# Jackxiini/Tensorflow-distributed-learning

Measured on AMD Instinct MI355X. Metric: images/sec (whole node) MNIST CNN global_batch=64*N, higher is better.
Workload: dtype fp32; 1 GPU; global_batch=64, parallelism=dp1, engine=fused, communicator=local, variant=reference, process_model=single, communicator_impl=LocalCommunicator, ipc_mode=dmabuf, allreduce=local, steps_per_execution=25, graph_captured=True, input_prefetch_executions=1, allreduce_in_graph=False, replicas_identical=True

## Files before the change

### csrc/kernels/mnist_cnn.hip

```cpp
#include <type_traits>

#include "common.h"
#include "mnist_cnn.h"
#include "optim.h"
#include "xgmi_device.h"

namespace tdl {

struct HeadWeights {
  float wa[10], wb[10], b4[10], b3a, b3b;
};

__device__ __forceinline__ HeadWeights load_head_weights(const MnistArgs& a, int l) {
  HeadWeights hw;
  const float* w4 = a.W + a.ow4;
#pragma unroll
  for (int c = 0; c < 10; ++c) {
    hw.wa[c] = w4[l * 10 + c];
    hw.wb[c] = w4[(l + 64) * 10 + c];
    hw.b4[c] = a.W[a.ob4 + c];
  }
  hw.b3a = a.W[a.ob3 + l];
  hw.b3b = a.W[a.ob3 + l + 64];
  return hw;
// ... 493 lines not shown
#pragma unroll
  for (int j = 0; j < 10; ++j) dw[j] = 0.f;
  const int d = 7 - wave;
  const int pix0 = half ? kDgSplit : 0, pix1 = half ? 169 : kDgSplit;
  if (d < (pix1 - pix0 + 15) / 16) {
    const int P = pix0 + d * 16 + i;
    const bool valid = P < pix1;
    const int Pc = valid ? P : pix0;
    const int ih = Pc / 13, iw = Pc - ih * 13;
    const float* wb = Wd + (g * 16 + i) * 4;
    const int c = 16 * h + i;
    unsigned q1v[4];
#pragma unroll
    for (int r = 0; r < 4; ++r) {
      const int Pr = min(pix0 + d * 16 + 4 * g + r, pix1 - 1);
      q1v[r] = a.A1[((size_t)bi * 169 + Pr) * 32 + c];
    }
    const int ih_lo = (pix0 + d * 16) / 13, ih_hi = min(pix0 + d * 16 + 15, pix1 - 1) / 13;
    const int kh_lo = max(0, ih_lo - 9), kh_hi = min(2, ih_hi);
    f4 acc0 = zero4(), acc1 = zero4();
    for (int kh = kh_lo; kh <= kh_hi; ++kh) {
#pragma unroll
      for (int kw = 0; kw < 3; ++kw) {
        const int tap = kh * 3 + kw;
        const float* ap = dCs + ((ih - kh + 2) * kDcDim + (iw - kw + 2)) * kDcStride + 4 * g;
#pragma unroll
        for (int c0 = 0; c0 < 64; c0 += 16) {
          const f4 av = ld4(ap + c0);
          const f4 bv = ld4(wb + (tap * 16 + c0 / 4) * 64);
          acc0 = mfma16x16x4(av.x, bv.x, acc0);
          acc1 = mfma16x16x4(av.y, bv.y, acc1);
          acc0 = mfma16x16x4(av.z, bv.z, acc0);
          acc1 = mfma16x16x4(av.w, bv.w, acc1);
        }
      }
    }
    const f4 acc = acc0 + acc1;
    stamp(a.stamps, 6);
#pragma unroll
    for (int r = 0; r < 4; ++r) {
      const int Pr = pix0 + d * 16 + 4 * g + r;
      if (Pr < pix1) {
        const float v = P1s[Pr * kP1StrideB + c] > 0.f ? acc[r] : 0.f;
        const unsigned q1 = q1v[r];
        const int ph = Pr / 13, pw = Pr - ph * 13;
        const float* img = Xs + (2 * ph + (q1 >> 1)) * 28 + 2 * pw + (q1 & 1);
#pragma unroll
        for (int kh = 0; kh < 3; ++kh)
#pragma unroll
          for (int kw = 0; kw < 3; ++kw) dw[kh * 3 + kw] = fmaf(img[kh * 28 + kw], v, dw[kh * 3 + kw]);
        dw[9] += v;
      }
    }
  }
#pragma unroll
  for (int j = 0; j < 10; ++j) dw[j] = sum_lane_groups(dw[j]);
  if (g == 0) {
#pragma unroll
    for (int j = 0; j < 10; ++j) red[(wave * 10 + j) * 16 + i] = dw[j];
  }
  stamp(a.stamps, 4);
  __syncthreads();
  stamp(a.stamps, 5);
  if (tid < 160) {
    const int j = tid >> 4, ii = tid & 15;
    float s = 0.f;
#pragma unroll
    for (int w = 2; w < 8; ++w) s += red[(w * 10 + j) * 16 + ii];
    a.part1[((size_t)bi * 2 + half) * kMnistPart1Cols + j * 32 + 16 * h + ii] = s;
  }
}

constexpr int kLdsFwd = 784 + 320 + 169 * kP1Stride + 72 * 16 * 4 + 400 + 169 * 32 / 4 + 400 / 4 + 16 * 128 + 4 + 128 +
                        288 * 16 +
                        kHeadW;
constexpr int kDcF = 15, kDcFStride = 20;
constexpr int kLdsFwdFused = kLdsFwd + kDcF * kDcF * kDcFStride;
constexpr int kP1Live = 12;
constexpr int kConv1Tiles = kP1Live * kP1Live / 4;
__constant__ int kFusedWgradTiles[8][2] = {{0, 2}, {3, 2}, {7, 3}, {12, 3}, {2, 1}, {5, 2}, {10, 2}, {15, 3}};

__device__ __forceinline__ void bwd_stamp(unsigned long long* buf, int k) {
  if (buf != nullptr && (threadIdx.x & 63) == 0)
    buf[(size_t)gridDim.x * 72 + (blockIdx.x * 8 + (threadIdx.x >> 6)) * 4 + k] = __builtin_amdgcn_s_memrealtime();
}

__device__ __forceinline__ void dgrad_mfma_stamp(unsigned long long* buf) {
#ifdef TDL_DIAG_DGRAD_STAMP
  if (buf != nullptr && (threadIdx.x & 63) == 0)
    buf[(size_t)gridDim.x * 104 + kFxBlocks * 16 + blockIdx.x * 8 + (threadIdx.x >> 6)] = __builtin_amdgcn_s_memrealtime();
#endif
}

constexpr int kWgS = 3;
struct FusedBwdPre {
  int wga[3], wgb;
  float wav[kWgS][3];
  int dga[3], xo[3][4];
  float p1v[3][4];
};

__device__ __forceinline__ int wg_wrap_a(int g) { return g >= 2 ? 3 * kP1Stride : 0; }

__device__ __forceinline__ void fused_bwd_pre(FusedBwdPre& pre, const float* P1s, const uint8_t* a1s) {
  const int wave = __builtin_amdgcn_readfirstlane(threadIdx.x >> 6), lane = threadIdx.x & 63;
  const int i = lane & 15, g = lane >> 4;
  const int t0 = kFusedWgradTiles[wave][0];
#pragma unroll
  for (int u = 0; u < 3; ++u) {
    const int k = min(t0 + u, 17) * 16 + i;
    const int tap = k >> 5, ci = k & 31;
    const int kh = tap / 3, kw = tap - kh * 3;
    pre.wga[u] = (kh * 13 + kw + g) * kP1Stride + ci;
  }
  pre.wgb = (2 * kDcF + 2 + g) * kDcFStride + i;
#pragma unroll
  for (int j = 0; j < kWgS; ++j) {
    const int q = (4 * j) / 10, r = (4 * j) % 10;
#pragma unroll
    for (int u = 0; u < 3; ++u) pre.wav[j][u] = P1s[pre.wga[u] + (q * 13 + r) * kP1Stride + (r == 8 ? wg_wrap_a(g) : 0)];
  }
  const int nt = wave >> 2, wt = wave & 3, ci = 16 * nt + i;
#pragma unroll
  for (int u = 0; u < 3; ++u) {
    const int t = wt + 4 * u;
    const int Pc = min(t * 16 + i, 168);
    const int ih = Pc / 13, iw = Pc - ih * 13;
    pre.dga[u] = ((ih + 2) * kDcF + iw + 2) * kDcFStride + 4 * g;
#pragma unroll
    for (int r = 0; r < 4; ++r) {
      const int Pr = min(t * 16 + 4 * g + r, 168);
      pre.p1v[u][r] = P1s[Pr * kP1Stride + ci];
      const int q1 = a1s[Pr * 32 + ci];
      const int ph = Pr / 13, pw = Pr - ph * 13;
      pre.xo[u][r] = (2 * ph + (q1 >> 1)) * 28 + 2 * pw + (q1 & 1);
    }
  }
}

template <int N>
__device__ __forceinline__ void fused_wgrad_tiles(const MnistArgs& a, int bi, int cq, int t0, const float* P1s,
                                                  const float* dCs, const FusedBwdPre& pre) {
  const int lane = threadIdx.x & 63, i = lane & 15, g = lane >> 4;
  const float* pa0[N];
#pragma unroll
  for (int u = 0; u < N; ++u) pa0[u] = P1s + pre.wga[u];
  const int wrapA = wg_wrap_a(g), wrapB = g >= 2 ? 5 * kDcFStride : 0;
  const float* pb0 = dCs + pre.wgb;
  f4 acc[N];
#pragma unroll
  for (int u = 0; u < N; ++u) acc[u] = zero4();
  constexpr int kS = kWgS, kBlocks = (25 + kS - 1) / kS;
  float bv[2][kS], av[2][kS][N];
  auto load = [&](int buf, int blk) {
#pragma unroll
    for (int j = 0; j < kS; ++j) {
      const int st = blk * kS + j;
      if (st >= 25) break;
      const int q = (4 * st) / 10, r = (4 * st) % 10;
      const bool strad = r == 8;
      bv[buf][j] = pb0[(q * kDcF + r) * kDcFStride + (strad ? wrapB : 0)];
#pragma unroll
      for (int u = 0; u < N; ++u)
        av[buf][j][u] = blk == 0 ? pre.wav[j][u] : pa0[u][(q * 13 + r) * kP1Stride + (strad ? wrapA : 0)];
    }
  };
  load(0, 0);
#pragma unroll
  for (int blk = 0; blk < kBlocks; ++blk) {
    if (blk + 1 < kBlocks) load((blk + 1) & 1, blk + 1);
    __builtin_amdgcn_sched_barrier(0);
#pragma unroll
    for (int j = 0; j < kS; ++j) {
      if (blk * kS + j >= 25) break;
#pragma unroll
      for (int u = 0; u < N; ++u) acc[u] = mfma16x16x4(av[blk & 1][j][u], bv[blk & 1][j], acc[u]);
    }
    __builtin_amdgcn_sched_barrier(0);
  }
  const auto rs = buf_rsrc(a.part2 + (size_t)bi * kP2QuadFloats, kP2QuadFloats * 4);
#pragma unroll
  for (int u = 0; u < N; ++u) st4_sc1(rs, ((((t0 + u) * 4 + g) * 64 + 16 * cq + i) * 4) * 4, acc[u]);
}

__device__ __forceinline__ void lds_dgrad_w2(const float* w2d, f4 (&bwd)[9]) {
  const int wave = __builtin_amdgcn_readfirstlane(threadIdx.x >> 6), lane = threadIdx.x & 63;
  const int i = lane & 15, g = lane >> 4, nt = wave >> 2;
#pragma unroll
  for (int tap = 0; tap < 9; ++tap) bwd[tap] = ld4(w2d + (tap * 32 + 16 * nt + i) * 16 + 4 * g);
}

constexpr int dg_kh_lo(int t) { return (16 * t) / 13 > 9 ? (16 * t) / 13 - 9 : 0; }
constexpr int dg_kh_hi(int t) { return (16 * t + 15) / 13 < 2 ? (16 * t + 15) / 13 : 2; }
constexpr int dg_taps(int t) { return 3 * (dg_kh_hi(t) - dg_kh_lo(t) + 1); }
static_assert(dg_taps(2) == 9 && dg_taps(3) == 9 && dg_taps(6) == 9 && dg_taps(7) == 9, "tile class 2");
static_assert(dg_taps(0) == 6 && dg_taps(4) == 9 && dg_taps(8) == 9 && dg_taps(1) == 9 && dg_taps(5) == 9 &&
              dg_taps(9) == 3, "tile classes 0 and 1");

#define TDL_SGB(mask, n) __builtin_amdgcn_sched_group_barrier(mask, n, 0)

template <int WTC>
__device__ __forceinline__ void fused_dgrad(const FusedBwdPre& pre, const float* dCs, const float* xs,
                                            const f4 (&bwd)[9], float (&dw)[10], unsigned long long* stamps) {
  constexpr int kT = WTC < 2 ? 3 : 2;
  auto lda = [&](int u, int tap) {
    const int kh = tap / 3, kw = tap - kh * 3;
    return ld4(dCs + pre.dga[u] - (kh * kDcF + kw) * kDcFStride);
  };
  auto ldx = [&](int u, int k, int r) { return xs[pre.xo[u][r] + (k / 3) * 28 + k % 3]; };
  f4 acc0 = zero4(), acc1 = zero4(), pacc0 = zero4(), pacc1 = zero4();
  float v[4] = {0.f, 0.f, 0.f, 0.f};
  f4 av[2];
  float ev[2][12];
  float el[9][4];
  av[0] = lda(0, 3 * dg_kh_lo(WTC));
  auto tile = [&](auto uc, auto sc) {
    constexpr int u = decltype(uc)::value, t = WTC + 4 * u, up = u > 0 ? u - 1 : 0;
    constexpr int s0 = decltype(sc)::value;
    constexpr int tap0 = 3 * dg_kh_lo(t), nA = dg_taps(t);
    constexpr int cps = u > 0 ? 9 / nA : 0;
    constexpr int lps = u + 1 == kT ? 9 / nA : 0;
    static_assert((u == 0 || cps * nA == 9) && (u + 1 < kT || lps * nA == 9), "epilogue split over the taps");
    acc0 = zero4();
    acc1 = zero4();
#pragma unroll
    for (int j = 0; j < nA; ++j) {
      const int p = (s0 + j) & 1;
      if (j + 1 < nA) {
        av[p ^ 1] = lda(u, tap0 + j + 1);
#pragma unroll
        for (int e = 0; e < 4 * cps; ++e) ev[p ^ 1][e] = ldx(up, (j + 1) * cps + (e >> 2), e & 3);
      } else if constexpr (u + 1 < kT) {
        constexpr int ncps = 9 / dg_taps(t + 4);
        av[p ^ 1] = lda(u + 1, 3 * dg_kh_lo(t + 4));
#pragma unroll
        for (int e = 0; e < 4 * ncps; ++e) ev[p ^ 1][e] = ldx(u, e >> 2, e & 3);
      }
#pragma unroll
      for (int e = 0; e < 4 * lps; ++e) el[j * lps + (e >> 2)][e & 3] = ldx(u, j * lps + (e >> 2), e & 3);
      __builtin_amdgcn_sched_barrier(0);
      const f4 x = av[p], bv = bwd[tap0 + j];
      auto fmas = [&](int first, int n) {
#pragma unroll
        for (int e = first; e < first + n; ++e) {
          const int k = j * cps + (e >> 2);
          dw[k] = fmaf(ev[p][e], v[e & 3], dw[k]);
        }
      };
      if (u > 0 && j == 0) {
        acc0 = mfma16x16x4(x.x, bv.x, acc0);
        acc1 = mfma16x16x4(x.y, bv.y, acc1);
        const f4 ac = pacc0 + pacc1;
#pragma unroll
        for (int r = 0; r < 4; ++r) {
          v[r] = pre.p1v[up][r] > 0.f ? ac[r] : 0.f;
          dw[9] += v[r];
        }
        acc0 = mfma16x16x4(x.z, bv.z, acc0);
        fmas(0, 2 * cps);
        acc1 = mfma16x16x4(x.w, bv.w, acc1);
        fmas(2 * cps, 2 * cps);
        TDL_SGB(0x8, 2);
        TDL_SGB(0x2, 16);
        TDL_SGB(0x8, 1);
        TDL_SGB(0x2, 2 * cps);
        TDL_SGB(0x8, 1);
        TDL_SGB(0x2, 2 * cps);
      } else {
        acc0 = mfma16x16x4(x.x, bv.x, acc0);
        fmas(0, cps);
        acc1 = mfma16x16x4(x.y, bv.y, acc1);
        fmas(cps, cps);
        acc0 = mfma16x16x4(x.z, bv.z, acc0);
        fmas(2 * cps, cps);
        acc1 = mfma16x16x4(x.w, bv.w, acc1);
        fmas(3 * cps, cps);
        if constexpr (cps > 0) {
#pragma unroll
          for (int m = 0; m < 4; ++m) {
            TDL_SGB(0x8, 1);
            TDL_SGB(0x2, cps);
          }
        }
      }
      __builtin_amdgcn_sched_barrier(0);
    }
    pacc0 = acc0;
    pacc1 = acc1;
  };
  constexpr int n0 = dg_taps(WTC), n1 = dg_taps(WTC + 4);
  tile(std::integral_constant<int, 0>{}, std::integral_constant<int, 0>{});
  tile(std::integral_constant<int, 1>{}, std::integral_constant<int, n0>{});
  if constexpr (kT == 3) tile(std::integral_constant<int, 2>{}, std::integral_constant<int, n0 + n1>{});
  dgrad_mfma_stamp(stamps);
  const f4 ac = pacc0 + pacc1;
#pragma unroll
  for (int r = 0; r < 4; ++r) {
    const float vl = pre.p1v[kT - 1][r] > 0.f ? ac[r] : 0.f;
#pragma unroll
    for (int k = 0; k < 9; ++k) dw[k] = fmaf(el[k][r], vl, dw[k]);
    dw[9] += vl;
  }
}
#undef TDL_SGB

__device__ __forceinline__ void fused_conv_bwd(const MnistArgs& a, int bi, int cq, const float* dp2s,
                                               const uint8_t* a2s, const float* P1s, const uint8_t* a1s,
                                               const float* xs, float* dCs, float* red, const f4 (&bwd)[9],
                                               FusedBwdPre& pre) {
  const int tid = threadIdx.x, wave = __builtin_amdgcn_readfirstlane(tid >> 6), lane = tid & 63;
  const int i = lane & 15, g = lane >> 4;
  bwd_stamp(a.stamps, 0);
  if (wave == 0) fused_bwd_pre(pre, P1s, a1s);

  auto wgrad = [&]() {
    const int t0 = kFusedWgradTiles[wave][0], ntiles = kFusedWgradTiles[wave][1];
    if (ntiles == 2) fused_wgrad_tiles<2>(a, bi, cq, t0, P1s, dCs, pre);
    else if (ntiles == 3) fused_wgrad_tiles<3>(a, bi, cq, t0, P1s, dCs, pre);
    else fused_wgrad_tiles<1>(a, bi, cq, t0, P1s, dCs, pre);
  };
  const bool swap = (a.variant & kMnistVariantStagger) && wave >= 4;
  if (!swap) wgrad();
  bwd_stamp(a.stamps, 1);

  float dw[10];
#pragma unroll
  for (int j = 0; j < 10; ++j) dw[j] = 0.f;
  const int wt = wave & 3;
  if (wt == 0) fused_dgrad<0>(pre, dCs, xs, bwd, dw, a.stamps);
  else if (wt == 1) fused_dgrad<1>(pre, dCs, xs, bwd, dw, a.stamps);
  else fused_dgrad<2>(pre, dCs, xs, bwd, dw, a.stamps);
  if (swap) wgrad();
  bwd_stamp(a.stamps, 2);
#pragma unroll
  for (int j = 0; j < 10; ++j) dw[j] = sum_lane_groups(dw[j]);
  if (g == 0) {
#pragma unroll
    for (int j = 0; j < 10; ++j) red[(wave * 10 + j) * 16 + i] = dw[j];
  }
  lds_barrier();
  bwd_stamp(a.stamps, 3);
  if (tid < kMnistPart1Cols) {
    const int j = tid >> 5, c = tid & 31, nt = c >> 4, ii = c & 15;
    float sum = 0.f;
#pragma unroll
    for (int w = 0; w < 4; ++w) sum += red[((4 * nt + w) * 10 + j) * 16 + ii];
    a.part1[((size_t)bi * 4 + cq) * kMnistPart1Cols + tid] = sum;
  }
}

__device__ __forceinline__ void store_saved_fwd(const MnistArgs& a, int bi, int cq, const float* P1s,
                                                const uint8_t* a1s, const float* p2s, const uint8_t* a2s,
                                                int t, int nt) {
  for (int e = (a.fused_bwd ? 676 : 0) + t; e < (a.fused_bwd ? 776 : 2 * 338 + 200); e += nt) {
    if (e < 338) {
      const int e4 = cq * 338 + e, pos = e4 >> 3, c4 = (e4 & 7) * 4;
      st4(a.P1 + (size_t)bi * 5408 + e4 * 4, ld4(P1s + pos * kP1Stride + c4));
    } else if (e < 676) {
      const int w = cq * 338 + (e - 338);
      reinterpret_cast<unsigned*>(a.A1 + (size_t)bi * 5408)[w] = reinterpret_cast<const unsigned*>(a1s)[w];
    } else if (e < 776) {
      const int u = e - 676, wo = u >> 2, q = u & 3;
      st4(a.P2 + (size_t)bi * 1600 + wo * 64 + 16 * cq + 4 * q, ld4(p2s + wo * 16 + 4 * q));
    } else {
      const int u = e - 776, wo = u >> 2, q = u & 3;
      *reinterpret_cast<unsigned*>(a.A2 + (size_t)bi * 1600 + wo * 64 + 16 * cq + 4 * q) =
          reinterpret_cast<const unsigned*>(a2s)[wo * 4 + q];
    }
  }
}

__global__ __launch_bounds__(512) void k_fwd_conv(MnistArgs a) {
  extern __shared__ __attribute__((aligned(16))) float sm[];
  float* xs = sm;
  float* w1s = xs + 784;
  float* P1s = w1s + 320;
  float* w2s = P1s + 169 * kP1Stride;
  float* p2s = w2s + 72 * 16 * 4;
  uint8_t* a1s = reinterpret_cast<uint8_t*>(p2s + 400);
  uint8_t* a2s = a1s + 169 * 32;
  float* red = reinterpret_cast<float*>(a2s + 400);
  int* s_last = reinterpret_cast<int*>(red + 16 * 128);
  float* w2d = red + 16 * 128 + 4 + 128;
  float* hws = w2d + 288 * 16;
  float* dCs = hws + kHeadW;
  const int tid = threadIdx.x, wave = tid >> 6, lane = tid & 63;
  const int i = lane & 15, g = lane >> 4;
  int bi = blockIdx.x >> 2, cq = blockIdx.x & 3;
  if ((a.variant & kMnistVariantXcd) && (a.b & 7) == 0) {
    const int x = blockIdx.x & 7, sl = blockIdx.x >> 3;
    bi = x * (a.b >> 3) + (sl >> 2);
    cq = sl & 3;
  }
  if ((a.variant & kMnistVariantPrio) && __builtin_amdgcn_readfirstlane(wave) >= 4) __builtin_amdgcn_s_setprio(1);
  stamp(a.stamps, 0);
  const int sample = a.idx[bi];
  const f4 vx = ld4(a.X + (size_t)sample * 784 + min(tid, 195) * 4);
  const int label = a.Y[sample];
  const float vw1 = tid < 288 ? a.W[a.ow1 + tid] : a.W[a.ob1 + min(tid - 288, 31)];
  f4 vw2[3];
#pragma unroll
  for (int j = 0; j < 3; ++j) {
    const int e = min(tid + j * 512, 1151);
    vw2[j] = ld4(a.W + a.ow2 + (e >> 2) * 64 + 16 * cq + (e & 3) * 4);
  }
  const float b2v = a.W[a.ob2 + 16 * cq + (lane & 15)];
  const uint32_t tag = a.ep[0] + 1u;
  __builtin_amdgcn_sched_barrier(0);
  if (tid < 196) st4(xs + tid * 4, vx);
  if (tid < 320) w1s[tid] = vw1;
#pragma unroll
  for (int j = 0; j < 3; ++j) {
    const int e = tid + j * 512;
    if (e < 1152) {
      const int k = e >> 2, q = e & 3;
      float* d = w2s + ((k >> 2) * 16 + 4 * q) * 4 + (k & 3);
      d[0] = vw2[j].x;
      d[4] = vw2[j].y;
      d[8] = vw2[j].z;
      d[12] = vw2[j].w;
      st4(w2d + k * 16 + 4 * q, vw2[j]);
    }
  }
  stamp(a.stamps, 1);
  __syncthreads();
  stamp(a.stamps, 2);
  const int n4 = (tid & 31) * 4, rg = tid >> 5;
  f4 w3v[25];
  const auto w3r = buf_rsrc(a.W + a.ow3 + (size_t)16 * cq * 128, (unsigned)((1600 - 16 * cq) * 128 * 4));
  const int w3vo = (rg * 128 + n4) * 4;
  auto ldw3 = [&](int j) { w3v[j] = ld4_buf(w3r, w3vo, j * 64 * 128 * 4); };
  auto ldw3_here = [&](int j) {
    __builtin_amdgcn_sched_barrier(0);
    ldw3(j);
    __builtin_amdgcn_sched_barrier(0);
  };
#pragma unroll
  for (int j = 0; j < 6; ++j) ldw3(j);
  {
    float bw[2][3];
#pragma unroll
    for (int nt = 0; nt < 2; ++nt)
#pragma unroll
      for (int s3 = 0; s3 < 3; ++s3) {
        const int k = 4 * s3 + g;
        bw[nt][s3] = k < 9 ? w1s[k * 32 + nt * 16 + i] : 0.f;
      }
    int tap_off[3];
#pragma unroll
    for (int s3 = 0; s3 < 3; ++s3) {
      const int k = min(4 * s3 + g, 8);
      tap_off[s3] = (k / 3) * 28 + (k % 3);
    }
    const float bias[2] = {w1s[288 + i], w1s[288 + 16 + i]};
    const int cwave = __builtin_amdgcn_readfirstlane(wave);
    static_assert(kConv1Tiles == 4 * 6 + 4 * 3, "slot -> tile map of conv1");
    auto live = [&](int it, int u) { return cwave < 4 || 2 * it + u < 3; };
    const int mtb = wave < 4 ? wave : 20 + wave;
    float xa[2][2][3];
    auto load_x = [&](int buf, int it) {
      const int mt0 = mtb + 8 * it;
#pragma unroll
      for (int u = 0; u < 2; ++u) {
        if (!live(it, u)) continue;
        const int w = (mt0 + 4 * u) * 4 + (i >> 2), q = i & 3;
        const int ph = w / kP1Live;
        const int y = 2 * ph + (q >> 1), x = 2 * (w - ph * kP1Live) + (q & 1);
        const float* xb = xs + y * 28 + x;
#pragma unroll
        for (int s3 = 0; s3 < 3; ++s3) xa[buf][u][s3] = xb[tap_off[s3]];
      }
    };
    load_x(0, 0);
#pragma unroll
    for (int it = 0; it < 3; ++it) {
      const int mt0 = mtb + 8 * it;
      f4 acc[2][2];
#pragma unroll
      for (int u = 0; u < 2; ++u)
#pragma unroll
        for (int nt = 0; nt < 2; ++nt) acc[u][nt] = zero4();
#pragma unroll
      for (int s3 = 0; s3 < 3; ++s3)
#pragma unroll
        for (int u = 0; u < 2; ++u) {
          if (live(it, u)) {
#pragma unroll
            for (int nt = 0; nt < 2; ++nt) acc[u][nt] = mfma16x16x4(xa[it & 1][u][s3], bw[nt][s3], acc[u][nt]);
          }
          if (it < 2 && 2 * s3 + u < 5) ldw3_here(6 + 5 * it + 2 * s3 + u);
        }
      __builtin_amdgcn_sched_barrier(0);
      if (it < 2) load_x((it + 1) & 1, it + 1);
      __builtin_amdgcn_sched_barrier(0);
#pragma unroll
      for (int u = 0; u < 2; ++u) {
        if (!live(it, u)) continue;
        const int w = (mt0 + 4 * u) * 4 + g;
        const int ph = w / kP1Live;
        const int wo = ph * 13 + (w - ph * kP1Live);
#pragma unroll
        for (int nt = 0; nt < 2; ++nt) {
          const f4 ac = acc[u][nt];
          float m = ac.x;
          unsigned am = 0;
          if (ac.y > m) { m = ac.y; am = 1; }
          if (ac.z > m) { m = ac.z; am = 2; }
          if (ac.w > m) { m = ac.w; am = 3; }
          const int co = nt * 16 + i;
          const float v = fmaxf(m + bias[nt], 0.f);
          P1s[wo * kP1Stride + co] = v;
          a1s[wo * 32 + co] = (uint8_t)am;
        }
      }
    }
    if (cwave >= 4) {
      const int e = tid - 256;
      if (e < 25 * 8) {
        const int c = e >> 3, c4 = e & 7;
        const int cell = c < 13 ? 12 * 13 + c : (c - 13) * 13 + 12;
        st4(P1s + cell * kP1Stride + 4 * c4, zero4());
        reinterpret_cast<unsigned*>(a1s)[cell * 8 + c4] = 0u;
      }
    }
  }
  stamp(a.stamps, 3);
  lds_barrier();
  stamp(a.stamps, 4);
  if (wave < 7) {
    const int wi = wave * 4 + (i >> 2), q = i & 3;
    const bool valid = wi < 25;
    const int wic = valid ? wi : 0;
    const int ph = wic / 5, pw = wic - ph * 5;
    const int oh = 2 * ph + (q >> 1), ow = 2 * pw + (q & 1);
    const float* ab = P1s + (oh * 13 + ow) * kP1Stride + 4 * g;
    const float* bb = w2s + (g * 16 + i) * 4;
    f4 acc0 = zero4(), acc1 = zero4();
#pragma unroll
    for (int kk = 0; kk < 9; ++kk) {
      const int kh = kk / 3, kw = kk % 3;
      f4 av[2], bv[2];
#pragma unroll
      for (int h = 0; h < 2; ++h) {
        av[h] = ld4(ab + (kh * 13 + kw) * kP1Stride + 16 * h);
        bv[h] = ld4(bb + ((kk * 32 + 16 * h) / 4) * 64);
      }
      ldw3_here(16 + kk);
#pragma unroll
      for (int h = 0; h < 2; ++h) {
        acc0 = mfma16x16x4(av[h].x, bv[h].x, acc0);
        acc1 = mfma16x16x4(av[h].y, bv[h].y, acc1);
        acc0 = mfma16x16x4(av[h].z, bv[h].z, acc0);
        acc1 = mfma16x16x4(av[h].w, bv[h].w, acc1);
      }
    }
    const f4 acc = acc0 + acc1;
    stamp(a.stamps, 5);
    const int wo = wave * 4 + g;
    if (wo < 25) {
      float m = acc.x;
      unsigned am = 0;
      if (acc.y > m) { m = acc.y; am = 1; }
      if (acc.z > m) { m = acc.z; am = 2; }
      if (acc.w > m) { m = acc.w; am = 3; }
      const float v = fmaxf(m + b2v, 0.f);
      p2s[wo * 16 + i] = v;
      a2s[wo * 16 + i] = (uint8_t)am;
    }
  } else {
#pragma unroll
    for (int j = 16; j < 25; ++j) ldw3(j);
    if (a.head != 0) {
      float hv[23];
#pragma unroll
      for (int u = 0; u < 23; ++u) {
        const int e = min(lane + 64 * u, 1417);
        hv[u] = a.W[e < 1280 ? a.ow4 + e : (e < 1408 ? a.ob3 + (e - 1280) : a.ob4 + (e - 1408))];
      }
#pragma unroll
      for (int u = 0; u < 23; ++u)
        if (lane + 64 * u < 1418) hws[lane + 64 * u] = hv[u];
    }
    if (a.head == 1 && a.dp2_fwd && a.fused_bwd) {
      for (int e4 = lane; e4 < kDcF * kDcF * kDcFStride / 4; e4 += 64) st4(dCs + e4 * 4, zero4());
    }
  }
  __syncthreads();
  {
    f4 hs = zero4();
#pragma unroll
    for (int j = 0; j < 25; ++j) hs += p2s[j * 16 + rg] * w3v[j];
    st4(red + rg * 128 + n4, hs);
  }
  lds_barrier();
  const bool tagged = a.head == 1 && a.dp2_fwd;
  float* sown = red + 16 * 128 + 4;
  if (tagged) {
    if (tid < 64) {
      typedef float f2 __attribute__((ext_vector_type(2)));
      f2 hsum = {0.f, 0.f};
#pragma unroll
      for (int k = 0; k < 16; ++k) hsum += *reinterpret_cast<const f2*>(red + k * 128 + 2 * tid);
      *reinterpret_cast<f2*>(sown + 2 * tid) = hsum;
      unsigned long long* p = a.part3t + ((size_t)cq * a.b + bi) * 128 + 2 * tid;
      const unsigned long long tg = (unsigned long long)tag << 32;
      __hip_atomic_store(p, (unsigned long long)__float_as_uint(hsum.x) | tg, __ATOMIC_RELAXED, __HIP_MEMORY_SCOPE_AGENT);
      __hip_atomic_store(p + 1, (unsigned long long)__float_as_uint(hsum.y) | tg, __ATOMIC_RELAXED,
                         __HIP_MEMORY_SCOPE_AGENT);
    }
  } else if (tid < 32) {
    f4 hsum = zero4();
#pragma unroll
    for (int k = 0; k < 16; ++k) hsum += ld4(red + k * 128 + 4 * tid);
    st4_sc1(buf_rsrc(a.part3 + ((size_t)cq * a.b + bi) * 128, 512), tid * 16, hsum);
  }
  stamp(a.stamps, 6);
  if (a.head == 0) {
    store_saved_fwd(a, bi, cq, P1s, a1s, p2s, a2s, tid, 512);
    return;
  }
  HeadWeights hw;
  const int uwave = __builtin_amdgcn_readfirstlane(wave);
  if (uwave == 0) hw = lds_head_weights(hws, lane);
  f4 bwd[9];
  const bool dgrad_w2 = a.head == 1 && a.dp2_fwd && a.fused_bwd;
  if (dgrad_w2 && uwave == 0) lds_dgrad_w2(w2d, bwd);

  if (!tagged) {
    asm volatile("s_waitcnt vmcnt(0)" ::: "memory");
    __syncthreads();
    if (tid == 0) {
      const unsigned old = __hip_atomic_fetch_add(a.cnt + bi, 1u, __ATOMIC_RELAXED, __HIP_MEMORY_SCOPE_AGENT);
      s_last[0] = (old & 3u) == 3u;
    }
  }
  lds_barrier();
  if (dgrad_w2 && uwave != 0) lds_dgrad_w2(w2d, bwd);
  const bool last = tagged || s_last[0] != 0;
  float* sdh = red;
  if (last && uwave == 0) {
    if (a.head == 1) head_row(a, bi, lane, label, hw, sdh, tag, tagged ? sown : nullptr, cq, !tagged || cq == kHeadQuarter);
    else head_eval(a, bi, lane, label, hw);
  }
  if (a.head != 1) return;
  if (!last) store_saved_fwd(a, bi, cq, P1s, a1s, p2s, a2s, tid, 512);
  else if (wave != 0) store_saved_fwd(a, bi, cq, P1s, a1s, p2s, a2s, tid - 64, 448);
  if (!a.dp2_fwd) return;
  FusedBwdPre pre;
  if (a.fused_bwd && uwave != 0) fused_bwd_pre(pre, P1s, a1s);
  lds_barrier();
  if (a.fused_bwd) stamp(a.stamps, 7);
  const f4 dh = ld4(sdh + n4);
  float v[25];
  {
    typedef float f2 __attribute__((ext_vector_type(2)));
    const f2 dlo = {dh.x, dh.y}, dhi = {dh.z, dh.w};
#pragma unroll
    for (int j = 0; j < 25; ++j) {
      f2 t = f2{w3v[j].x, w3v[j].y} * dlo;
      t = __builtin_elementwise_fma(f2{w3v[j].z, w3v[j].w}, dhi, t);
      v[j] = t.x + t.y;
    }
  }
  const float d = reduce_scatter32<25>(v, lane);
  const int j = lane & 31;
  if (a.fused_bwd) {
    float val = 0.f;
    if (j < 25) {
      const int kk = j * 16 + rg;
      val = p2s[kk] > 0.f ? d : 0.f;
      const unsigned am = a2s[kk];
      const int ph = (j * 13) >> 6, pw = j - 5 * ph;
      const int y = 2 * ph + (int)(am >> 1), x = 2 * pw + (int)(am & 1u);
      dCs[((y + 2) * kDcF + x + 2) * kDcFStride + rg] = val;
    }
    float sb = rs_swap16(val, val);
    sb += dpp_xor8(sb);
    sb += dpp_mirror8(sb);
    sb += dpp_xor2(sb);
    sb += dpp_xor1(sb);
    if (j == 0) {
      const auto rs = buf_rsrc(a.part2 + (size_t)bi * kP2QuadFloats, kP2QuadFloats * 4);
      st4_sc1(rs, (((kP2Quads - 1) * 64 + 16 * cq + rg) * 4) * 4, f4{sb, 0.f, 0.f, 0.f});
    }
    lds_barrier();
    fused_conv_bwd(a, bi, cq, p2s, a2s, P1s, a1s, xs, dCs, red, bwd, pre);
    return;
  }
  if (j < 25) {
    const int kk = j * 16 + rg;
    a.dP2[(size_t)bi * 1600 + j * 64 + 16 * cq + rg] = p2s[kk] > 0.f ? d : 0.f;
  }
  stamp(a.stamps, 7);
}

__global__ __launch_bounds__(256) void k_finalize(MnistArgs a, int apply_sgd, int ndb, int nbs, int nb2, int nb1) {
  const float lr = *a.lr;
  int blk = blockIdx.x;
  if (blk < ndb) {
    const int T = blk * 4 + (threadIdx.x >> 6);
    if (T < kDenseTasks) dense_w_task(a, T, threadIdx.x & 63, apply_sgd != 0, lr);
    return;
  }
  blk -= ndb;
  if (blk < nbs) {
    const int e = a.ow3 + blk * 256 + threadIdx.x;
    if (e < a.nslab) a.W[e] -= lr * a.G[e];
    return;
  }
  if (blk < nbs + nb2) {
    const int t = (blk - nbs) * 256 + threadIdx.x;
    const int o = t >> 2, sub = t & 3;
    const int n = kMnistPart2Rows * 64;
    float s = 0.f;
    const int oc = min(o, n - 1);
    const int e = (oc >> 6) < 288 ? a.ow2 + oc : a.ob2 + (oc & 63);
    const float wold = apply_sgd ? a.W[e] : 0.f;
    for (int base = 0; base < a.b; base += 64) {
      float v[16];
#pragma unroll
      for (int j = 0; j < 16; ++j) v[j] = a.part2[(size_t)min(base + sub + 4 * j, a.b - 1) * n + oc];
#pragma unroll
      for (int j = 0; j < 16; ++j) s += (base + sub + 4 * j < a.b) ? v[j] : 0.f;
    }
    s += __shfl_xor(s, 1, 64);
    s += __shfl_xor(s, 2, 64);
    if (sub == 0 && o < n) {
      a.G[e] = s;
      if (apply_sgd) a.W[e] = wold - lr * s;
    }
    return;
  }
  const int t = (blk - nbs - nb2) * 256 + threadIdx.x;
  const int o = t >> 4, sub = t & 15;
  const int rows = mnist_part1_rows(a.b, a.fused_bwd != 0);
  float s = 0.f;
  const int oc = min(o, kMnistPart1Cols - 1);
  const int e = oc < 288 ? a.ow1 + oc : a.ob1 + (oc - 288);
  const float wold = apply_sgd ? a.W[e] : 0.f;
  for (int base = 0; base < rows; base += 128) {
    float v[8];
#pragma unroll
    for (int j = 0; j < 8; ++j) v[j] = a.part1[(size_t)min(base + sub + 16 * j, rows - 1) * kMnistPart1Cols + oc];
#pragma unroll
    for (int j = 0; j < 8; ++j) s += (base + sub + 16 * j < rows) ? v[j] : 0.f;
  }
#pragma unroll
  for (int m = 1; m < 16; m <<= 1) s += __shfl_xor(s, m, 64);
  if (sub == 0 && o < kMnistPart1Cols) {
    a.G[e] = s;
    if (apply_sgd) a.W[e] = wold - lr * s;
  }
}

__device__ __forceinline__ void fx_range(const MnistArgs& a, int j, int& lo, int& cnt, int& nseg, int& stride) {
  nseg = 1;
  stride = 0;
  if (j < kFxW3) {
    lo = a.ow3 + (j >> 1) * 2048 + (j & 1) * 64;
    cnt = 64;
    nseg = 16;
    stride = 128;
  } else if (j < kFxW3 + 4) {
    lo = a.ob3 + 32 * (j - kFxW3);
    cnt = 32;
  } else if (j < kFxW3 + 8) {
    lo = a.ow4 + 320 * (j - kFxW3 - 4);
    cnt = 320;
  } else if (j == kFxW3 + 8) {
    lo = a.ob4;
    cnt = 10;
  } else if (j < kFxDense + kFxConv2) {
    const int qd = (j - kFxDense) >> 1, h = (j - kFxDense) & 1;
    if (qd == kP2Quads - 1) {
      lo = a.ob2 + 32 * h;
      cnt = 32;
    } else {
      lo = a.ow2 + qd * 256 + 32 * h;
      cnt = 32;
      nseg = 4;
      stride = 64;
    }
  } else {
    const int q = j - kFxDense - kFxConv2;
    lo = q < 18 ? a.ow1 + q * 16 : a.ob1 + (q - 18) * 16;
    cnt = 16;
  }
}

template <int R>
__device__ __forceinline__ void finalize_x_body(const MnistArgs& a, int apply_sgd, int j);

template <int R, bool LOOP>
__global__ __launch_bounds__(512) void k_finalize_x(MnistArgs a, int apply_sgd) {
  unsigned long long* sb = a.stamps == nullptr ? nullptr
      : a.stamps + (size_t)a.b * 4 * 104 + ((size_t)blockIdx.x * 8 + (threadIdx.x >> 6)) * 2;
  if (sb != nullptr && (threadIdx.x & 63) == 0) sb[0] = __builtin_amdgcn_s_memrealtime();
  if constexpr (LOOP) {
    for (int j = blockIdx.x; j < kFxBlocks; j += gridDim.x) {
      finalize_x_body<R>(a, apply_sgd, j);
      __syncthreads();
    }
  } else {
    finalize_x_body<R>(a, apply_sgd, blockIdx.x);
  }
  if (sb != nullptr && (threadIdx.x & 63) == 0) sb[1] = __builtin_amdgcn_s_memrealtime();
}

template <int R>
__device__ __forceinline__ void finalize_x_body(const MnistArgs& a, int apply_sgd, int j) {
  const int tid = threadIdx.x, wave = tid >> 6, lane = tid & 63;
  const float lr = *a.lr;
  const bool xchg = R > 1 && a.xchg && apply_sgd;
  if (j == 0 && tid == 4 * 64) a.ep[0] += 1u;
  uint32_t e = 0;
  float* xdst = nullptr;
  int64_t half = 0;
  if (xchg) {
// ... 294 lines not shown
```

Before: 2.862 million images/sec.

## Software-pipeline conv1 MFMA with previous-tile epilogue and deferred w2 LDS stores

Restructures the conv1 forward loop into a per-tile software pipeline in which the maxpool/ReLU epilogue of the previous tile is interleaved with the MFMAs of the current tile using sched_group_barrier hints. Address offsets for inputs and outputs are precomputed into registers before the barrier. The w2 LDS staging stores are moved past the barrier into the pipeline, and __syncthreads is replaced by lds_barrier. This aims to hide epilogue ALU and LDS latency behind MFMA work, at the cost of more live registers, hardcoded LDS byte offsets, and a w2 store ordering that must still complete before its consumers.

```diff
diff --git a/csrc/kernels/mnist_cnn.hip b/csrc/kernels/mnist_cnn.hip
--- a/csrc/kernels/mnist_cnn.hip
+++ b/csrc/kernels/mnist_cnn.hip
@@ -819,7 +819,6 @@
     dw[9] += vl;
   }
 }
-#undef TDL_SGB
 
 __device__ __forceinline__ void fused_conv_bwd(const MnistArgs& a, int bi, int cq, const float* dp2s,
                                                const uint8_t* a2s, const float* P1s, const uint8_t* a1s,
@@ -923,11 +922,27 @@
   }
   const float b2v = a.W[a.ob2 + 16 * cq + (lane & 15)];
   const uint32_t tag = a.ep[0] + 1u;
+  const int c1mtb = wave < 4 ? wave : 20 + wave;
+  int c1x[6], c1p[6], c1a[6];
+#pragma unroll
+  for (int s = 0; s < 6; ++s) {
+    const int mt = c1mtb + 4 * (wave < 4 ? s : min(s, 2));
+    const int w = mt * 4 + (i >> 2), q = i & 3;
+    const int ph = w / kP1Live;
+    c1x[s] = ((2 * ph + (q >> 1)) * 28 + 2 * (w - ph * kP1Live) + (q & 1)) * 4;
+    const int we = mt * 4 + g;
+    const int pe = we / kP1Live;
+    const int wo = pe * 13 + (we - pe * kP1Live);
+    c1p[s] = (784 + 320 + wo * kP1Stride + i) * 4;
+    c1a[s] = (784 + 320 + 169 * kP1Stride + 72 * 16 * 4 + 400) * 4 + wo * 32 + i;
+    asm volatile("" : "+v"(c1x[s]), "+v"(c1p[s]), "+v"(c1a[s]));
+  }
+  int c1t0 = ((g / 3) * 28 + g % 3) * 4, c1t1 = (((4 + g) / 3) * 28 + (4 + g) % 3) * 4;
+  asm volatile("" : "+v"(c1t0), "+v"(c1t1));
   __builtin_amdgcn_sched_barrier(0);
   if (tid < 196) st4(xs + tid * 4, vx);
   if (tid < 320) w1s[tid] = vw1;
-#pragma unroll
-  for (int j = 0; j < 3; ++j) {
+  auto st_w2 = [&](int j) {
     const int e = tid + j * 512;
     if (e < 1152) {
       const int k = e >> 2, q = e & 3;
@@ -938,9 +953,9 @@
       d[12] = vw2[j].w;
       st4(w2d + k * 16 + 4 * q, vw2[j]);
     }
-  }
+  };
   stamp(a.stamps, 1);
-  __syncthreads();
+  lds_barrier();
   stamp(a.stamps, 2);
   const int n4 = (tid & 31) * 4, rg = tid >> 5;
   f4 w3v[25];
@@ -963,74 +978,80 @@
         const int k = 4 * s3 + g;
         bw[nt][s3] = k < 9 ? w1s[k * 32 + nt * 16 + i] : 0.f;
       }
-    int tap_off[3];
-#pragma unroll
-    for (int s3 = 0; s3 < 3; ++s3) {
-      const int k = min(4 * s3 + g, 8);
-      tap_off[s3] = (k / 3) * 28 + (k % 3);
-    }
     const float bias[2] = {w1s[288 + i], w1s[288 + 16 + i]};
     const int cwave = __builtin_amdgcn_readfirstlane(wave);
     static_assert(kConv1Tiles == 4 * 6 + 4 * 3, "slot -> tile map of conv1");
-    auto live = [&](int it, int u) { return cwave < 4 || 2 * it + u < 3; };
-    const int mtb = wave < 4 ? wave : 20 + wave;
-    float xa[2][2][3];
-    auto load_x = [&](int buf, int it) {
-      const int mt0 = mtb + 8 * it;
-#pragma unroll
-      for (int u = 0; u < 2; ++u) {
-        if (!live(it, u)) continue;
-        const int w = (mt0 + 4 * u) * 4 + (i >> 2), q = i & 3;
-        const int ph = w / kP1Live;
-        const int y = 2 * ph + (q >> 1), x = 2 * (w - ph * kP1Live) + (q & 1);
-        const float* xb = xs + y * 28 + x;
-#pragma unroll
-        for (int s3 = 0; s3 < 3; ++s3) xa[buf][u][s3] = xb[tap_off[s3]];
-      }
+    auto conv1_pipe = [&](auto nsc) {
+      constexpr int NS = decltype(nsc)::value;
+      const char* smb = reinterpret_cast<const char*>(sm);
+      float xa[2][3];
+      auto load_x = [&](int s) {
+        const char* p = smb + c1x[s];
+        xa[s & 1][0] = *reinterpret_cast<const float*>(p + c1t0);
+        xa[s & 1][1] = *reinterpret_cast<const float*>(p + c1t1);
+        xa[s & 1][2] = *reinterpret_cast<const float*>(p + (2 * 28 + 2) * 4);
+      };
+      f4 pacc[2] = {zero4(), zero4()};
+      float m[2];
+      unsigned am[2];
+      auto epi = [&](int s, int p) {
+        const int nt = p / 3;
+        const f4 ac = pacc[nt];
+        if (p % 3 == 0) {
+          m[nt] = ac.x;
+          am[nt] = 0;
+          if (ac.y > m[nt]) { m[nt] = ac.y; am[nt] = 1; }
+        } else if (p % 3 == 1) {
+          if (ac.z > m[nt]) { m[nt] = ac.z; am[nt] = 2; }
+        } else {
+          if (ac.w > m[nt]) { m[nt] = ac.w; am[nt] = 3; }
+          const float v = fmaxf(m[nt] + bias[nt], 0.f);
+          char* smw = reinterpret_cast<char*>(sm);
+          *reinterpret_cast<float*>(smw + c1p[s] + nt * 64) = v;
+          *reinterpret_cast<uint8_t*>(smw + c1a[s] + nt * 16) = (uint8_t)am[nt];
+        }
+      };
+      load_x(0);
+#pragma unroll
+      for (int s = 0; s < NS; ++s) {
+        if (s + 1 < NS) load_x(s + 1);
+        if (s < 3) st_w2(s);
+        __builtin_amdgcn_sched_barrier(0);
+        f4 acc[2] = {zero4(), zero4()};
+#pragma unroll
+        for (int s3 = 0; s3 < 3; ++s3) {
+          acc[0] = mfma16x16x4(xa[s & 1][s3], bw[0][s3], acc[0]);
+          if (s > 0) epi(s - 1, 2 * s3);
+          acc[1] = mfma16x16x4(xa[s & 1][s3], bw[1][s3], acc[1]);
+          if (s > 0) epi(s - 1, 2 * s3 + 1);
+          if (s > 0) {
+            TDL_SGB(0x8, 1);
+            if (s3 == 1) {
+              TDL_SGB(0x2, 5);
+              TDL_SGB(0x200, 2);
+            } else {
+              TDL_SGB(0x2, 3);
+            }
+            TDL_SGB(0x8, 1);
+            if (s3 == 2) {
+              TDL_SGB(0x2, 5);
+              TDL_SGB(0x200, 2);
+            } else {
+              TDL_SGB(0x2, 3);
+            }
+          }
+          if (3 * s + s3 < 10) ldw3_here(6 + 3 * s + s3);
+          else __builtin_amdgcn_sched_barrier(0);
+        }
+        pacc[0] = acc[0];
+        pacc[1] = acc[1];
+      }
+      if (NS == 3) ldw3_here(15);
+#pragma unroll
+      for (int p = 0; p < 6; ++p) epi(NS - 1, p);
     };
-    load_x(0, 0);
-#pragma unroll
-    for (int it = 0; it < 3; ++it) {
-      const int mt0 = mtb + 8 * it;
-      f4 acc[2][2];
-#pragma unroll
-      for (int u = 0; u < 2; ++u)
-#pragma unroll
-        for (int nt = 0; nt < 2; ++nt) acc[u][nt] = zero4();
-#pragma unroll
-      for (int s3 = 0; s3 < 3; ++s3)
-#pragma unroll
-        for (int u = 0; u < 2; ++u) {
-          if (live(it, u)) {
-#pragma unroll
-            for (int nt = 0; nt < 2; ++nt) acc[u][nt] = mfma16x16x4(xa[it & 1][u][s3], bw[nt][s3], acc[u][nt]);
-          }
-          if (it < 2 && 2 * s3 + u < 5) ldw3_here(6 + 5 * it + 2 * s3 + u);
-        }
-      __builtin_amdgcn_sched_barrier(0);
-      if (it < 2) load_x((it + 1) & 1, it + 1);
-      __builtin_amdgcn_sched_barrier(0);
-#pragma unroll
-      for (int u = 0; u < 2; ++u) {
-        if (!live(it, u)) continue;
-        const int w = (mt0 + 4 * u) * 4 + g;
-        const int ph = w / kP1Live;
-        const int wo = ph * 13 + (w - ph * kP1Live);
-#pragma unroll
-        for (int nt = 0; nt < 2; ++nt) {
-          const f4 ac = acc[u][nt];
-          float m = ac.x;
-          unsigned am = 0;
-          if (ac.y > m) { m = ac.y; am = 1; }
-          if (ac.z > m) { m = ac.z; am = 2; }
-          if (ac.w > m) { m = ac.w; am = 3; }
-          const int co = nt * 16 + i;
-          const float v = fmaxf(m + bias[nt], 0.f);
-          P1s[wo * kP1Stride + co] = v;
-          a1s[wo * 32 + co] = (uint8_t)am;
-        }
-      }
-    }
+    if (cwave < 4) conv1_pipe(std::integral_constant<int, 6>{});
+    else conv1_pipe(std::integral_constant<int, 3>{});
     if (cwave >= 4) {
       const int e = tid - 256;
       if (e < 25 * 8) {
```

Result: no change. 2.889 million images/sec, median of 6 (+1.0%).
